# ngrabaskas/Torch-Automatic-Distributed-Neural-Network

Measured on AMD Instinct MI355X. Metric: samples/sec whole-node ResNet-50 DP + GPT-2 PP at 1/2/4/8 MI355X; scaling eff, higher is better.
Workload: dtype bf16

## Files before the change

madnn/models/resnet.py:

```python
from __future__ import annotations

import os
from typing import List, Optional, Type

import torch
from torch import nn

from ..nn.conv import FusedConv2d
from ..nn.norm import FusedBatchNorm2d as BN
from ..nn.norm import FusedGlobalAvgPool2d, FusedMaxPool2d
from ..ops import (batch_norm_add_bn_relu, bn_relu_conv1x1, bn_relu_conv1x1_epi_supported,
                   bn_relu_conv3x3, conv1x1_route,
                   bn_relu_conv3x3_supported, bn_relu_maxpool, bn_relu_maxpool_supported)

_FORK_DS = os.environ.get("MADNN_FORK_DOWNSAMPLE", "1") != "0"
_DUAL_BN = os.environ.get("MADNN_DUAL_BN", "1") != "0"
_DS_SUB = os.environ.get("MADNN_DS_SUB", "1") != "0"


def conv3x3(cin, cout, stride=1, groups=1, dilation=1):
    return FusedConv2d(cin, cout, 3, stride=stride, padding=dilation, groups=groups, bias=False, dilation=dilation)


def conv1x1(cin, cout, stride=1):
    return FusedConv2d(cin, cout, 1, stride=stride, bias=False)


class BasicBlock(nn.Module):
    expansion = 1

    def __init__(self, inplanes, planes, stride=1, downsample=None):
        super().__init__()
        self.conv1 = conv3x3(inplanes, planes, stride)
        self.bn1 = BN(planes)
        self.conv2 = conv3x3(planes, planes)
# ... 22 lines not shown
        self.downsample = downsample

    def forward(self, x):
        if self.downsample is None:
            y, st, idt = self.conv1(x, stats=True, fork=True)
            if isinstance(idt, torch.Tensor) and isinstance(self.bn3, BN) and self.conv1._k9(x) \
                    and conv1x1_route(x.size(1), self.conv1.weight.size(0))[1] == "k9":
                idt._madnn_defer_mask = True
        elif _FORK_DS:
            dual = self._dual_bn()
            sub = dual and _DS_SUB and isinstance(x, torch.Tensor) and self.downsample[0].subsampled_ok()
            y, st, xf = self.conv1(x, stats=True, fork=2 if sub else True)
            if dual:
                yd, std = (self.downsample[0].forward_subsampled(xf, stats=True) if sub
                           else self.downsample[0](xf, stats=True))
                y, st = self._bn1_conv2(y, st)
                y, st = self._bn2_conv3(y, st)
                return batch_norm_add_bn_relu(y, yd, self.bn3, self.downsample[1], st, std)
            idt = self.downsample(xf)
        else:
            idt = self.downsample(x)
            y, st = self.conv1(x, stats=True)
        y, st = self._bn1_conv2(y, st)
        y, st = self._bn2_conv3(y, st)
        return self.bn3(y, residual=idt, relu=True, stats=st)

    def _bn1_conv2(self, y, st):
        if isinstance(y, torch.Tensor) and isinstance(self.bn1, BN) and isinstance(self.conv2, FusedConv2d) \
                and self.conv2._k13(y) \
                and bn_relu_conv3x3_supported(y, self.bn1, self.conv2.weight):
            return bn_relu_conv3x3(y, self.bn1, self.conv2.weight, stats_in=st, stats=True)
        out = self.bn1(y, relu=True, stats=st)
        return self.conv2(out, stats=True)

    def _bn2_conv3(self, y, st):
        if isinstance(y, torch.Tensor) and isinstance(self.bn2, BN) and isinstance(self.conv3, FusedConv2d) \
                and self.conv3._k9(y) and bn_relu_conv1x1_epi_supported(y, self.bn2, self.conv3.weight):
            return bn_relu_conv1x1(y, self.bn2, self.conv3.weight, stats_in=st, stats=True)
        out = self.bn2(y, relu=True, stats=st)
        return self.conv3(out, stats=True)

    def _dual_bn(self) -> bool:
        ds = self.downsample
        return (_DUAL_BN and isinstance(ds, nn.Sequential) and len(ds) == 2
                and isinstance(ds[0], FusedConv2d) and isinstance(ds[1], BN) and isinstance(self.bn3, BN))

# ... 82 lines not shown
```

madnn/ops/__init__.py:

```python
from __future__ import annotations

import os
import threading
from pathlib import Path
from typing import Optional, Sequence

import torch
import torch.nn.functional as F

from . import reference

HERE = Path(__file__).resolve().parent
_KERNELS = HERE / "_madnn_kernels.so"
_lock = threading.Lock()
_loaded = {"kernels": False, "error": None}


def kernels_path() -> Path:
    return _KERNELS


class StaleKernelsError(RuntimeError):
    """The in-tree kernel library was built from different sources than the tree holds."""

# ... 708 lines not shown


def bn_relu_conv1x1(y: torch.Tensor, bn, w: torch.Tensor, *, stats_in: Optional[torch.Tensor] = None,
                    stats: bool = False):
    if bn_relu_conv1x1_epi_supported(y, bn, w):
        _need_native("bn_relu_conv1x1")
        out, part = _BNReluConv1x1EpiFn.apply(y, w, bn.weight, bn.bias, bn, stats_in, stats)
        return (out, part if part.numel() else None) if stats else out
    a = bn(y, relu=True, stats=stats_in) if _is_fused_bn(bn) else torch.relu(bn(y))
    if conv1x1_supported(a, w):
        return conv1x1(a, w, stats=stats)
    out = torch.nn.functional.conv2d(a, w.view(w.size(0), -1, 1, 1)) if a.dim() == 4 else torch.mm(
        a, w.reshape(w.size(0), -1).t())
    return (out, None) if stats else out


def bn_relu_conv1x1_epi_supported(y: torch.Tensor, bn, w: torch.Tensor) -> bool:
    return (_BN_DGRAD_EPI and isinstance(y, torch.Tensor) and bn.training and bn.track_running_stats
            and bn.affine and bn.momentum is not None and bn.weight.dtype == torch.float32
            and conv1x1_supported(y, w) and bn_supported(y, bn.weight)
            and conv1x1_route(y.size(1), w.size(0))[1] == "k9")


class _BNReluMaxPoolFn(torch.autograd.Function):

    @staticmethod
    def forward(ctx, y, bn_w, bn_b, bn, stats_in, p):
        mean, invstd, scale, shift = torch.ops.madnn.bn_coef(y, bn_w, bn_b, bn.running_mean, bn.running_var,
                                                             bn.num_batches_tracked, float(bn.momentum),
                                                             float(bn.eps), stats_in)
        out, arg = torch.ops.madnn.pool_bn_fwd(y, scale, shift, int(p))
        ctx.save_for_backward(y, arg, bn_w, mean, invstd, scale, shift)
        ctx.p = int(p)
        return out

    @staticmethod
    def backward(ctx, dp):
        y, arg, bn_w, mean, invstd, scale, shift = ctx.saved_tensors
        dy, dw, db = torch.ops.madnn.pool_bn_bwd(dp, arg, y, bn_w, mean, invstd, scale, shift, ctx.p)
        return dy, dw, db, None, None, None


def bn_relu_maxpool_supported(y: torch.Tensor, bn, pool) -> bool:
    def pair(v):
        return tuple(v) if isinstance(v, (tuple, list)) else (v, v)
    return (_POOL_BN and isinstance(y, torch.Tensor) and y.device.type == "cuda" and y.dtype == torch.bfloat16 and y.dim() == 4
# ... 211 lines not shown
        if ctx.needs_input_grad[1]:
            dw = torch.ops.madnn.stem_wgrad(dy, x).to(w.dtype)
            if not dw.is_contiguous(memory_format=torch.contiguous_format) or w.stride() != dw.stride():
                dw = torch.empty_like(w).copy_(dw)
        return dx, dw, None


def stem_conv(x: torch.Tensor, w: torch.Tensor, *, stats: bool = False):
    _need_native("stem_conv")
    y, part = _StemFn.apply(x, w, stats)
    return (y, part) if stats else y


def hidden_supported(h: int) -> bool:
    return h % 8 == 0 and h <= 16384


__all__ = [
    "bucket_pack", "bucket_unpack", "flat_scale_cast", "sgd_step", "adam_step", "grad_norm", "layer_norm",
    "rms_norm", "batch_norm_act", "bn_supported", "cross_entropy", "attention", "attention_qkvpacked", "attention_supported",
    "max_pool2d", "max_pool_supported", "conv1x1", "conv1x1_route", "batch_norm_add_bn_relu",
    "batch_norm_dual_supported", "bn_relu_conv1x1", "bn_relu_maxpool",
    "bn_relu_maxpool_supported", "bn_relu_conv3x3", "bn_relu_conv3x3_supported",
    "bn_relu_conv1x1_epi_supported", "conv1x1_supported", "stem_conv", "stem_supported", "native_available", "load_kernels", "kernels_path", "hidden_supported", "reference",
]

if os.environ.get("MADNN_EAGER_LOAD", "0") == "1":
    load_kernels()


FUSED_LINEAR = os.environ.get("MADNN_FUSED_LINEAR", "1") != "0"

def _gelu_tanh_grad(p: torch.Tensor) -> torch.Tensor:
    k0, k1 = 0.7978845608028654, 0.044715
    t = torch.tanh(k0 * (p + k1 * p * p * p))
    return 0.5 * (1 + t) + 0.5 * p * (1 - t * t) * k0 * (1 + 3 * k1 * p * p)


GELU_KIND = {"tanh": 1, "none": 2}


def _gelu_grad_ref(p: torch.Tensor, kind: int) -> torch.Tensor:
    if kind == 1:
        return _gelu_tanh_grad(p)
    cdf = 0.5 * (1.0 + torch.erf(p * 0.7071067811865476))
    return cdf + p * torch.exp(-0.5 * p * p) * 0.3989422804014327

# ... 548 lines not shown
```

madnn/ops/csrc/binding.cpp:

```cpp
#include <torch/library.h>
#include <ATen/ATen.h>
#include <ATen/hip/impl/HIPGuardImplMasqueradingAsCUDA.h>
#include <ATen/hip/impl/HIPStreamMasqueradingAsCUDA.h>
#include <hip/hip_runtime.h>

#include <vector>

#include "attn.h"

extern "C" {
hipError_t madnn_bucket_pack(void* const*, const int64_t*, const int64_t*, int, void*, int, int, float, hipStream_t);
hipError_t madnn_bucket_unpack(void* const*, const int64_t*, const int64_t*, int, void*, int, int, float, hipStream_t);
hipError_t madnn_flat_scale_cast(const void*, void*, int64_t, int, int, float, hipStream_t);
hipError_t madnn_sgd_step(float*, const void*, int, float*, void*, int, int64_t, float, float, float, float, int, int,
                          float, const float*, hipStream_t);
hipError_t madnn_adam_step(float*, const void*, int, float*, float*, void*, int, int64_t, float, float, float, float,
                           float, int, float, float, float, const float*, hipStream_t);
int madnn_sqnorm_grid(int64_t);
hipError_t madnn_sqnorm_partial(const void*, int, int64_t, float, float*, int, hipStream_t);
hipError_t madnn_norm_finalize(const float*, int, float, float*, hipStream_t);
hipError_t madnn_norm_fwd(const void*, const void*, const void*, const void*, void*, void*, float*, float*, int64_t,
                          int, float, int, int, int, hipStream_t);
int64_t madnn_norm_bwd_workspace(int64_t, int);
hipError_t madnn_norm_bwd(const void*, const void*, const void*, const float*, const float*, const void*, void*, void*,
// ... 24 lines not shown
hipError_t madnn_pool_bn_bwd(const void*, const void*, const void*, const float*, const float*, const float*,
                             const float*, const float*, void*, float*, float*, float*, float*, int, int, int, int, int,
                             int, int, hipStream_t);
hipError_t madnn_maxpool_bwd(const void*, const void*, void*, int, int, int, int, int, int, int, int, int, int,
                             hipStream_t);
hipError_t madnn_xent_fwd(const void*, int, const int64_t*, int64_t, int64_t, int64_t, int, int, float*, float*,
                          hipStream_t);
hipError_t madnn_xent_bwd(const void*, int, const int64_t*, const float*, int64_t, int64_t, int64_t, int, int, int64_t,
                          const float*, void*, hipStream_t);
int madnn_xent_fused_chunks(int64_t);
hipError_t madnn_xent_fused(const void*, int, const int64_t*, int64_t, int64_t, int64_t, int, int, int64_t,
                            const float*, float*, void*, hipStream_t);
hipError_t madnn_xent_rescale(void*, int, int64_t, const float*, hipStream_t);
hipError_t madnn_bn_bwd(const void*, const void*, const unsigned char*, int, void*, void*, int64_t, int, int, int,
                        const float*, const float*, const float*, const float*, const float*, float*, float*, float*,
                        float*, hipStream_t);
hipError_t madnn_bn_fwd_dual(const void*, const void*, void*, unsigned char*, int64_t, int, float, float, const float*,
                             const float*, float*, float*, int64_t*, float*, float*, float*, float*, const float*, int,
                             float, float, const float*, const float*, float*, float*, int64_t*, float*, float*,
                             float*, float*, const float*, int, float*, hipStream_t);
hipError_t madnn_bn_bwd_dual(const void*, const void*, const void*, const unsigned char*, void*, void*, int64_t, int,
                             const float*, const float*, const float*, const float*, const float*, const float*,
                             float*, float*, float*, float*, float*, float*, hipStream_t);
int madnn_conv1x1_supported(int64_t, int64_t);
int madnn_conv1x1_stat_rows(int64_t, int64_t, int64_t);
hipError_t madnn_conv1x1_fwd(const void*, const void*, void*, float*, int64_t, int64_t, int64_t, hipStream_t);
hipError_t madnn_conv1x1_dgrad(const void*, const void*, void*, const void*, int64_t, int64_t, int64_t, const void*,
                               const float*, const float*, float*, hipStream_t, const unsigned char* = nullptr);
int madnn_conv1x1_dgrad_rows(int64_t, int64_t, int64_t);
int64_t madnn_conv1x1_wgrad_ws(int64_t, int64_t, int64_t);
hipError_t madnn_conv1x1_wgrad(const void*, const void*, void*, int, float*, int64_t, int64_t, int64_t, hipStream_t);
hipError_t madnn_bn_coef(const void*, int64_t, int, float, float, const float*, const float*, float*, float*, int64_t*,
                         float*, float*, float*, float*, float*, const float*, int, hipStream_t);
int madnn_stem_supported(int, int);
int madnn_stem_stat_rows(int, int, int);
hipError_t madnn_stem_fwd(const void*, const void*, void*, float*, int, int, int, hipStream_t);
int64_t madnn_stem_wgrad_ws(int, int, int);
hipError_t madnn_stem_wgrad(const void*, const void*, float*, float*, int, int, int, hipStream_t);
int madnn_gemm_supported(int64_t, int64_t, int64_t, int64_t, int64_t);
int madnn_conv3x3_supported(int, int, int, int);
int madnn_conv3x3_stat_rows(int64_t);
hipError_t madnn_conv3x3_fwd(const void*, const void*, void*, float*, int, int, int, int, int, hipStream_t);
int madnn_conv3x3_s2_supported(int, int, int, int);
int madnn_conv3x3_s2_stat_rows(int, int, int);
hipError_t madnn_conv3x3_fwd_s2(const void*, const void*, void*, float*, int, int, int, int, int, hipStream_t);
int64_t madnn_conv3x3_wgrad_ws(int, int, int, int, int);
// ... 528 lines not shown
  at::hip::HIPGuardMasqueradingAsCUDA guard(dy.device());
  at::Tensor dx = conv_out_like(dy, cin);
  at::Tensor part = at::empty({madnn_conv1x1_dgrad_rows(M, cin, cout), 2, cin}, dy.options().dtype(at::kFloat));
  check(madnn_conv1x1_dgrad(dy.data_ptr(), w.data_ptr(), dx.data_ptr(), nullptr, M, cin, cout, bny.data_ptr(),
                            scale.data_ptr<float>(), shift.data_ptr<float>(), part.data_ptr<float>(), cur_stream(dy)),
        "conv1x1_dgrad_bnb");
  return {dx, part};
}

at::Tensor conv1x1_wgrad(const at::Tensor& dy, const at::Tensor& x, bool out_bf16) {
  const int64_t cout = dy.size(1), cin = x.size(1);
  const int64_t M = conv_rows(x, cin, "x");
  TORCH_CHECK(conv_rows(dy, cout, "dy") == M && dy.dim() == x.dim(), "conv1x1_wgrad: dy / x pixel mismatch");
  TORCH_CHECK(madnn_conv1x1_supported(cin, cout), "conv1x1: channels must be multiples of 64");
  at::hip::HIPGuardMasqueradingAsCUDA guard(x.device());
  at::Tensor dw = at::empty({cout, cin}, x.options().dtype(out_bf16 ? at::kBFloat16 : at::kFloat));
  at::Tensor ws = at::empty({madnn_conv1x1_wgrad_ws(M, cin, cout)}, x.options().dtype(at::kFloat));
  check(madnn_conv1x1_wgrad(dy.data_ptr(), x.data_ptr(), dw.data_ptr(), out_bf16 ? 1 : 0, ws.data_ptr<float>(), M, cin,
                            cout, cur_stream(x)),
        "conv1x1_wgrad");
  return dw;
}

void gemm_check(const at::Tensor& t, const char* name) {
  check_dev(t, name);
  TORCH_CHECK(t.scalar_type() == at::kBFloat16, "linear: ", name, " must be bf16");
  TORCH_CHECK(t.is_contiguous(), "linear: ", name, " must be contiguous");
  TORCH_CHECK(reinterpret_cast<uintptr_t>(t.data_ptr()) % 16 == 0, "linear: ", name, " must be 16-B aligned");
}

std::tuple<at::Tensor, at::Tensor> linear_fwd(const at::Tensor& x, const at::Tensor& w,
                                              const c10::optional<at::Tensor>& bias,
                                              const c10::optional<at::Tensor>& res, int64_t act, bool save_aux) {
  gemm_check(x, "x");
  gemm_check(w, "w");
  const int64_t K = x.size(-1), N = w.size(0), M = x.numel() / std::max<int64_t>(K, 1);
  TORCH_CHECK(w.dim() == 2 && w.size(1) == K, "linear: weight must be [N, K]");
  TORCH_CHECK(madnn_gemm_supported(N, M, K, K, K), "linear: unsupported shape M=", M, " N=", N, " K=", K);
  at::hip::HIPGuardMasqueradingAsCUDA guard(x.device());
  std::vector<int64_t> shape(x.sizes().begin(), x.sizes().end());
  shape.back() = N;
  at::Tensor y = at::empty(shape, x.options());
  at::Tensor aux = save_aux ? at::empty(shape, x.options()) : at::empty({0}, x.options());
  const bool hb = bias.has_value() && bias->defined();
  if (hb) {
    check_dev(*bias, "bias");
// ... 719 lines not shown
      "bn_bwd(Tensor dy, Tensor x, Tensor? mask, bool has_res, Tensor? w, Tensor save_mean, Tensor save_invstd, "
      "Tensor scale, Tensor shift, bool relu, bool need_wgrad, bool write_dres=True) -> (Tensor, Tensor, Tensor, Tensor)");
  m.def(
      "bn_fwd_dual(Tensor x, Tensor r, Tensor? w, Tensor? b, Tensor(a!)? run_mean, Tensor(b!)? run_var, "
      "Tensor(c!)? nbt, float momentum, float eps, Tensor? partial, Tensor? w_r, Tensor? b_r, "
      "Tensor(d!)? run_mean_r, Tensor(e!)? run_var_r, Tensor(f!)? nbt_r, float momentum_r, float eps_r, "
      "Tensor? partial_r) -> Tensor[]");
  m.def(
      "bn_bwd_dual(Tensor dy, Tensor x, Tensor r, Tensor mask, Tensor? w, Tensor save_mean, Tensor save_invstd, "
      "Tensor? w_r, Tensor save_mean_r, Tensor save_invstd_r) -> Tensor[]");
  m.def("attn_fwd(Tensor q, Tensor k, Tensor v, bool causal, float scale) -> (Tensor, Tensor)");
  m.def(
      "attn_bwd(Tensor dout, Tensor q, Tensor k, Tensor v, Tensor o, Tensor lse, Tensor(a!) dq, Tensor(b!) dk, "
      "Tensor(c!) dv, bool causal, float scale, Tensor(d!)? colsum=None) -> ()");
  m.def("conv1x1_fwd(Tensor x, Tensor w, bool stats) -> (Tensor, Tensor)");
  m.def("conv1x1_dgrad(Tensor dy, Tensor w, Tensor? res=None, Tensor? resmask=None) -> Tensor");
  m.def("conv1x1_dgrad_bnb(Tensor dy, Tensor w, Tensor bny, Tensor scale, Tensor shift) -> (Tensor, Tensor)");
  m.def(
      "conv3x3_fwd_bnb(Tensor x, Tensor w, Tensor bny, Tensor scale, Tensor shift) -> (Tensor, Tensor)");
  m.def(
      "bn_bwd_ext(Tensor dy, Tensor x, Tensor? w, Tensor save_mean, Tensor save_invstd, Tensor scale, Tensor shift, "
      "Tensor partial, bool relu) -> (Tensor, Tensor, Tensor)");
  m.def("conv1x1_wgrad(Tensor dy, Tensor x, bool out_bf16=False) -> Tensor");
  m.def(
      "bn_coef(Tensor x, Tensor? w, Tensor? b, Tensor(a!)? run_mean, Tensor(b!)? run_var, Tensor(c!)? nbt, "
      "float momentum, float eps, Tensor? partial=None) -> Tensor[]");
  m.def("stem_fwd(Tensor x, Tensor wp, bool stats) -> (Tensor, Tensor)");
  m.def("linear_fwd(Tensor x, Tensor w, Tensor? bias, Tensor? res, int act, bool save_aux) -> (Tensor, Tensor)");
  m.def("linear_dgrad(Tensor dy, Tensor w, Tensor? res, bool accumulate) -> Tensor");
  m.def("linear_wgrad(Tensor dy, Tensor x, Tensor? out, bool accumulate, int splits) -> Tensor");
  m.def("linear_wgrad4(Tensor dy, Tensor x, Tensor? out, bool accumulate, int splits) -> Tensor");
  m.def("linear_wgrad4h(Tensor dy, Tensor x, Tensor? out, bool accumulate, int splits) -> Tensor");
  m.def("wgrad_splits(int M, int N, int K) -> int", &wgrad_splits);
  m.def("gemmp_supported(int I, int J, int K, bool has_bias) -> bool", &gemmp_supported);
  m.def("linear_fwd_p(Tensor x, Tensor w, Tensor? bias, int act) -> (Tensor, Tensor)");
  m.def("linear_dgrad_p(Tensor dy, Tensor w, Tensor? pre, ScalarType bias_dtype, int gelu_kind=1) -> (Tensor, Tensor)");
  m.def("conv3x3_fwd(Tensor x, Tensor w, bool stats) -> (Tensor, Tensor)");
  m.def("conv3x3_fwd_s2(Tensor x, Tensor w, bool stats) -> (Tensor, Tensor)");
  m.def("conv3x3_wgrad(Tensor dy, Tensor x, bool out_bf16) -> Tensor");
  m.def("stem_wgrad(Tensor dy, Tensor x) -> Tensor");
  m.def("bias_grad(Tensor dy, Tensor? pre, ScalarType bias_dtype, int gelu_kind=1) -> (Tensor, Tensor)");
  m.def("gelu_fwd(Tensor x, int kind=1) -> Tensor");
  m.def("rope_qkv_(Tensor(a!) qkv, Tensor cos, Tensor sin, int rot_heads, bool inverse) -> Tensor(a!)");
  m.def("rope_qkv(Tensor qkv, Tensor cos, Tensor sin, int rot_heads, bool inverse) -> Tensor");
  m.def("swiglu_fwd(Tensor gu) -> Tensor");
  m.def("swiglu_bwd(Tensor dh, Tensor gu) -> Tensor");
// ... 36 lines not shown
  m.impl("conv3x3_fwd_bnb", conv3x3_fwd_bnb);
  m.impl("conv1x1_dgrad_bnb", conv1x1_dgrad_bnb);
  m.impl("bn_bwd_ext", bn_bwd_ext);
  m.impl("bn_bwd_dual", bn_bwd_dual);
  m.impl("xent_fwd", xent_fwd);
  m.impl("xent_bwd", xent_bwd);
  m.impl("xent_fused", xent_fused);
  m.impl("xent_rescale", xent_rescale);
  m.impl("maxpool_fwd", maxpool_fwd);
  m.impl("pool_bn_fwd", pool_bn_fwd);
  m.impl("pool_bn_bwd", pool_bn_bwd);
  m.impl("bias_grad", bias_grad);
  m.impl("gelu_fwd", gelu_fwd);
  m.impl("rope_qkv_", rope_qkv_);
  m.impl("rope_qkv", rope_qkv);
  m.impl("swiglu_fwd", swiglu_fwd);
  m.impl("swiglu_bwd", swiglu_bwd);
  m.impl("attn_fwd", attn_fwd);
  m.impl("attn_bwd", attn_bwd);
  m.impl("maxpool_bwd", maxpool_bwd);
  m.impl("conv1x1_fwd", conv1x1_fwd);
  m.impl("conv1x1_dgrad", conv1x1_dgrad);
  m.impl("conv1x1_wgrad", conv1x1_wgrad);
  m.impl("stem_fwd", stem_fwd);
  m.impl("stem_wgrad", stem_wgrad);
  m.impl("linear_fwd", linear_fwd);
  m.impl("linear_dgrad", linear_dgrad);
  m.impl("linear_wgrad", linear_wgrad);
  m.impl("linear_wgrad4", linear_wgrad4);
  m.impl("linear_wgrad4h", linear_wgrad4h);
  m.impl("linear_fwd_p", linear_fwd_p);
  m.impl("linear_dgrad_p", linear_dgrad_p);
  m.impl("conv3x3_fwd", conv3x3_fwd);
  m.impl("conv3x3_fwd_s2", conv3x3_fwd_s2);
  m.impl("conv3x3_wgrad", conv3x3_wgrad);
  m.impl("hwq_wait", hwq_wait);
  m.impl("hwq_set", hwq_set);
  m.impl("hwq_batch", hwq_batch);
  m.impl("hwq_spin", hwq_spin);
}
```

madnn/ops/csrc/bn.hip:

```cpp
#include <type_traits>

#include "common.h"

namespace madnn {

constexpr int kBnThreads = 256;
constexpr int kFinSlices = 32;

struct BnGeom {
  int tpr, rpi;
};

struct BnTune {
  int reverse = 1;
  int wg_per_cu = 3;
  int hoist = 1;
  int partials_per_cu = 2;
};
inline BnTune& bn_tune() {
  static BnTune t;
  return t;
}
inline int bn_walk_flags() { return (bn_tune().reverse ? 1 : 0) | (bn_tune().hoist ? 0 : 2); }

// ... 501 lines not shown
      part = prereduce(ext_partial, G, C, ps, qo, workspace, stream);
    } else {
      MADNN_DISPATCH_DT(xdt, XDT, {
        hipLaunchKernelGGL((bn_stats_kernel<XDT>), dim3(G), dim3(kBnThreads), lds, stream, x, M, C, workspace);
      });
      MADNN_HIP_CHECK(hipGetLastError());
    }
    hipLaunchKernelGGL(bn_stats_finalize_kernel, dim3((C + 31) / 32), dim3(32 * kFinSlices), 0, stream, part, G, C, M, eps,
                       momentum, w, b, save_mean, save_invstd, scale, shift, run_mean, run_var, nbt);
  } else {
    hipLaunchKernelGGL(bn_eval_coef_kernel, dim3((C + 255) / 256), dim3(256), 0, stream, C, eps, w, b, run_mean,
                       run_var, scale, shift);
  }
  MADNN_HIP_CHECK(hipGetLastError());
  const int64_t total = M * C;
  const int grid = stream_grid(total, 256 * 8, bn_tune().wg_per_cu * kNumCU);
  MADNN_DISPATCH_DT(xdt, XDT, MADNN_BN_VARIANT(relu, res != nullptr, RELU, RES, {
    hipLaunchKernelGGL((bn_apply_kernel<XDT, RELU, RES>), dim3(grid), dim3(256), 0, stream, x, res, scale, shift, y,
                       mask, total, C, bn_walk_flags());
  }));
  return hipGetLastError();
}

hipError_t madnn_bn_bwd(const void* dy, const void* x, const unsigned char* mask, int has_res, void* dx, void* dres,
                        int64_t M, int C, int xdt, int relu, const float* w, const float* save_mean,
                        const float* save_invstd, const float* scale, const float* shift, float* dw, float* db,
                        float* coef, float* workspace, hipStream_t stream) {
  using namespace madnn;
  if (!madnn_bn_supported(C)) return hipErrorInvalidValue;
  if (M <= 0) return hipSuccess;
  const int G = bn_grid_rows(M, C);
  const BnGeom g = bn_geom(C);
  const size_t lds = g.rpi > 1 ? (size_t)g.rpi * 2 * C * sizeof(float) : 0;
  if (relu && has_res && mask == nullptr) return hipErrorInvalidValue;
  MADNN_DISPATCH_DT(xdt, XDT, MADNN_BN_VARIANT(relu, has_res, RELU, RES, {
    hipLaunchKernelGGL((bn_bwd_reduce_kernel<XDT, RELU, RELU && RES>), dim3(G), dim3(kBnThreads), lds, stream, dy, x,
                       mask, scale, shift, M, C, workspace);
  }));
  MADNN_HIP_CHECK(hipGetLastError());
  float* ca = coef;
  float* cb = coef + C;
  float* cc = coef + 2 * C;
  hipLaunchKernelGGL(bn_bwd_finalize_kernel, dim3((C + 31) / 32), dim3(32 * kFinSlices), 0, stream, workspace, G, C, 2 * C, C, M, w,
                     save_mean, save_invstd, dw, db, ca, cb, cc);
  MADNN_HIP_CHECK(hipGetLastError());
  const int64_t total = M * C;
  const int grid = stream_grid(total, 256 * 8, bn_tune().wg_per_cu * kNumCU);
  MADNN_DISPATCH_DT(xdt, XDT, MADNN_BN_VARIANT(relu, has_res, RELU, RES, {
    hipLaunchKernelGGL((bn_bwd_apply_kernel<XDT, RELU, RES>), dim3(grid), dim3(256), 0, stream, dy, x, mask, scale,
                       shift, ca, cb, cc, dx, dres, total, C, bn_walk_flags());
  }));
  return hipGetLastError();
}


hipError_t madnn_bn_fwd_dual(const void* x, const void* r, void* y, unsigned char* mask, int64_t M, int C,
                             float eps, float momentum, const float* w, const float* b, float* run_mean,
                             float* run_var, int64_t* nbt, float* save_mean, float* save_invstd, float* scale,
                             float* shift, const float* ext_partial, int ext_rows, float eps_r, float momentum_r,
                             const float* w_r, const float* b_r, float* run_mean_r, float* run_var_r,
                             int64_t* nbt_r, float* save_mean_r, float* save_invstd_r, float* scale_r,
                             float* shift_r, const float* ext_partial_r, int ext_rows_r, float* workspace,
                             hipStream_t stream) {
  using namespace madnn;
  if (!madnn_bn_supported(C) || mask == nullptr) return hipErrorInvalidValue;
  if (M <= 0) return hipSuccess;
  const BnGeom g = bn_geom(C);
  const size_t lds = g.rpi > 1 ? (size_t)g.rpi * 2 * C * sizeof(float) : 0;
// ... 124 lines not shown
```

madnn/ops/csrc/conv.hip:

```cpp
#include "mfma.h"

namespace madnn {
namespace conv {

using namespace mf;

constexpr int kThreads = 256;
constexpr int kBK = 64;
constexpr int kTargetWG = 2 * kNumCU;

struct Tune {
  int fwd_wg = kTargetWG;
  int wgrad_wg = 2 * kNumCU;
  int xcd = 1;
};
inline Tune& tune() {
  static Tune t;
  return t;
}

enum Mode : int { kStoreT = 0, kSplit = 1 };

struct GemmArgs {
  const uint16_t* a;
// ... 296 lines not shown
  for (int64_t v = (int64_t)blockIdx.x * 256 + threadIdx.x; v < n4; v += (int64_t)gridDim.x * 256) {
    f32x4 acc = reinterpret_cast<const f32x4*>(slab)[v];
    for (int s = 1; s < splits; ++s) acc += reinterpret_cast<const f32x4*>(slab + (int64_t)s * n)[v];
    if constexpr (BF16) {
      const unsigned lo = (unsigned)f32_to_bf16(acc[0]) | ((unsigned)f32_to_bf16(acc[1]) << 16);
      const unsigned hi = (unsigned)f32_to_bf16(acc[2]) | ((unsigned)f32_to_bf16(acc[3]) << 16);
      reinterpret_cast<u32x2*>(dw)[v] = u32x2{lo, hi};
    } else {
      reinterpret_cast<f32x4*>(dw)[v] = acc;
    }
  }
}

inline void wgrad_split(int64_t M, int64_t cin, int64_t cout, int& bi, int& bj, int64_t& tiles, int& k_chunk,
                        int64_t& splits) {
  bi = cout % 128 == 0 ? 128 : 64;
  bj = cin % 128 == 0 ? 128 : 64;
  tiles = (cout / bi) * (cin / bj);
  const int64_t nk = (M + kBK - 1) / kBK;
  splits = (tune().wgrad_wg + tiles - 1) / tiles;
  splits = splits < 1 ? 1 : (splits > nk ? nk : splits);
  k_chunk = (int)((nk + splits - 1) / splits);
  splits = (nk + k_chunk - 1) / k_chunk;
}

}
}

using namespace madnn::conv;

extern "C" {

int madnn_conv1x1_tune(int key, int value) {
  int* f = key == 0 ? &tune().fwd_wg : key == 1 ? &tune().wgrad_wg : key == 2 ? &tune().xcd : nullptr;
  if (f == nullptr) return -1;
  const int old = *f;
  if (value >= 0) *f = value;
  return old;
}

int madnn_conv1x1_supported(int64_t cin, int64_t cout) {
  return (cin % 64 == 0 && cout % 64 == 0 && cin >= 64 && cout >= 64 && cin <= 16384 && cout <= 16384) ? 1 : 0;
}

int madnn_conv1x1_stat_rows(int64_t M, int64_t cin, int64_t cout) {
  if (!madnn_conv1x1_supported(cin, cout) || M <= 0) return 0;
// ... 97 lines not shown
  if (ws == nullptr) return hipErrorInvalidValue;
  p.out = ws;
  p.i_tiles = (int)(cout / bi);
  p.j_tiles = (int)(cin / bj);
  const int grid = (int)(tiles * splits);
  p.j_groups = 0;
  hipError_t e;
  if (bi == 128 && bj == 128) e = launch<true, true, 128, 128, kSplit, false>(p, grid, s);
  else if (bi == 128) e = launch<true, true, 128, 64, kSplit, false>(p, grid, s);
  else if (bj == 128) e = launch<true, true, 64, 128, kSplit, false>(p, grid, s);
  else e = launch<true, true, 64, 64, kSplit, false>(p, grid, s);
  if (e != hipSuccess) return e;
  const int64_t n = cin * cout;
  const int64_t blocks = (n / 4 + 255) / 256;
  const dim3 grid_r((unsigned)(blocks < 4 * madnn::kNumCU ? blocks : 4 * madnn::kNumCU));
  if (dw_bf16) {
    hipLaunchKernelGGL(split_reduce_kernel<true>, grid_r, dim3(256), 0, s, ws, (int)splits, n, dw);
  } else {
    hipLaunchKernelGGL(split_reduce_kernel<false>, grid_r, dim3(256), 0, s, ws, (int)splits, n, dw);
  }
  return hipGetLastError();
}

}
```

Baseline: 13440.

## Fuse bn3 backward apply, conv3 dgrad/wgrad and bn2 stats into one kernel

Adds an autograd function for non-downsample bottleneck blocks with 64->256 channels that chains bn2, conv3 and bn3+residual+ReLU in the forward pass. In the backward pass, a new HIP kernel applies the bn3 backward coefficients to dout on the fly and computes conv3 dgrad and wgrad together from one pass over the tile. It also accumulates the bn2 backward partial sums in its epilogue, so the bn3 dx tensor is never materialised and the separate dgrad, wgrad and stats passes are removed. The cost is a specialised kernel that only handles C=64 (layer1), a per-workgroup fp32 weight-gradient slab buffer that needs a split-reduce, and more complexity in the backward path.

```diff
diff --git a/madnn/models/resnet.py b/madnn/models/resnet.py
--- a/madnn/models/resnet.py
+++ b/madnn/models/resnet.py
@@ -9,8 +9,8 @@
 from ..nn.conv import FusedConv2d
 from ..nn.norm import FusedBatchNorm2d as BN
 from ..nn.norm import FusedGlobalAvgPool2d, FusedMaxPool2d
-from ..ops import (batch_norm_add_bn_relu, bn_relu_conv1x1, bn_relu_conv1x1_epi_supported,
-                   bn_relu_conv3x3, conv1x1_route,
+from ..ops import (batch_norm_add_bn_relu, bn2_conv3_bn3_add_relu, bn2_conv3_bn3_supported, bn_relu_conv1x1,
+                   bn_relu_conv1x1_epi_supported, bn_relu_conv3x3, conv1x1_route,
                    bn_relu_conv3x3_supported, bn_relu_maxpool, bn_relu_maxpool_supported)
 
 _FORK_DS = os.environ.get("MADNN_FORK_DOWNSAMPLE", "1") != "0"
@@ -79,6 +79,10 @@
             idt = self.downsample(x)
             y, st = self.conv1(x, stats=True)
         y, st = self._bn1_conv2(y, st)
+        if self.downsample is None and isinstance(self.bn2, BN) and isinstance(self.bn3, BN) \
+                and isinstance(self.conv3, FusedConv2d) and isinstance(y, torch.Tensor) and self.conv3._k9(y) \
+                and bn2_conv3_bn3_supported(y, self.bn2, self.conv3.weight, self.bn3, idt):
+            return bn2_conv3_bn3_add_relu(y, self.bn2, self.conv3.weight, self.bn3, idt, stats_in=st)
         y, st = self._bn2_conv3(y, st)
         return self.bn3(y, residual=idt, relu=True, stats=st)
 
diff --git a/madnn/ops/__init__.py b/madnn/ops/__init__.py
--- a/madnn/ops/__init__.py
+++ b/madnn/ops/__init__.py
@@ -754,6 +754,63 @@
             and conv1x1_route(y.size(1), w.size(0))[1] == "k9")
 
 
+class _BN2Conv3BN3Fn(torch.autograd.Function):
+
+    @staticmethod
+    def forward(ctx, y2, w3, bn2_w, bn2_b, bn3_w, bn3_b, idt, bn2, bn3, stats_in):
+        a2, mean2, invstd2, scale2, shift2, _ = torch.ops.madnn.bn_fwd(
+            y2, None, bn2_w, bn2_b, bn2.running_mean, bn2.running_var, bn2.num_batches_tracked, True,
+            float(bn2.momentum), float(bn2.eps), True, stats_in)
+        y3, part = torch.ops.madnn.conv1x1_fwd(a2, w3, True)
+        out, mean3, invstd3, scale3, shift3, mask = torch.ops.madnn.bn_fwd(
+            y3, idt, bn3_w, bn3_b, bn3.running_mean, bn3.running_var, bn3.num_batches_tracked, True,
+            float(bn3.momentum), float(bn3.eps), True, part)
+        ctx.save_for_backward(y2, a2, w3, y3, mask, bn2_w, mean2, invstd2, scale2, shift2, bn3_w, mean3, invstd3,
+                              scale3, shift3)
+        return out
+
+    @staticmethod
+    def backward(ctx, dout):
+        (y2, a2, w3, y3, mask, bn2_w, mean2, invstd2, scale2, shift2, bn3_w, mean3, invstd3, scale3,
+         shift3) = ctx.saved_tensors
+        if dout.dtype != y3.dtype or dout.stride() != y3.stride():
+            dout = torch.empty_like(y3).copy_(dout)
+        coef, dbw3, dbb3 = torch.ops.madnn.bn_bwd_coef(dout, y3, mask, bn3_w, mean3, invstd3, scale3, shift3)
+        da2, part, dw3 = torch.ops.madnn.bn3_conv3_bwd(dout, y3, mask, coef, w3, a2, y2, scale2, shift2,
+                                                       w3.dtype == torch.bfloat16)
+        dy2, dbw2, dbb2 = torch.ops.madnn.bn_bwd_ext(da2, y2, bn2_w, mean2, invstd2, scale2, shift2, part, True)
+        dres = dout.view_as(dout)
+        _attach(dres, "_madnn_resmask", mask)
+        need2 = ctx.needs_input_grad[2] or ctx.needs_input_grad[3]
+        need3 = ctx.needs_input_grad[4] or ctx.needs_input_grad[5]
+        return (dy2, dw3.to(w3.dtype).view(w3.shape), dbw2 if need2 else None, dbb2 if need2 else None,
+                dbw3 if need3 else None, dbb3 if need3 else None, dres, None, None, None)
+
+
+_BN3_CONV3_FUSED = os.environ.get("MADNN_BN3_CONV3_FUSED", "1") != "0"
+
+
+def bn2_conv3_bn3_supported(y2: torch.Tensor, bn2, w3: torch.Tensor, bn3, idt: torch.Tensor) -> bool:
+    def ok(m):
+        return (m.training and m.track_running_stats and m.affine and m.momentum is not None
+                and m.weight.dtype == torch.float32)
+    if not (_BN3_CONV3_FUSED and DEFER_RES_MASK and isinstance(y2, torch.Tensor) and isinstance(idt, torch.Tensor)):
+        return False
+    c, c4 = y2.size(1), w3.size(0)
+    return (bn_relu_conv1x1_epi_supported(y2, bn2, w3) and native_available()
+            and bool(torch.ops.madnn.bn3_conv3_bwd_supported(c, c4)) and conv1x1_route(c, c4)[0] == "k9" and ok(bn2) and ok(bn3)
+            and bn3.weight.numel() == c4 and y2.requires_grad and torch.is_grad_enabled()
+            and getattr(idt, "_madnn_defer_mask", False) and idt.dtype == y2.dtype and idt.dim() == y2.dim()
+            and idt.size(1) == c4 and idt.shape[2:] == y2.shape[2:] and idt.size(0) == y2.size(0)
+            and bn_supported(idt, bn3.weight))
+
+
+def bn2_conv3_bn3_add_relu(y2: torch.Tensor, bn2, w3: torch.Tensor, bn3, idt: torch.Tensor,
+                           stats_in: Optional[torch.Tensor] = None) -> torch.Tensor:
+    _need_native("bn2_conv3_bn3_add_relu")
+    return _BN2Conv3BN3Fn.apply(y2, w3, bn2.weight, bn2.bias, bn3.weight, bn3.bias, idt, bn2, bn3, stats_in)
+
+
 class _BNReluMaxPoolFn(torch.autograd.Function):
 
     @staticmethod
@@ -1011,7 +1068,7 @@
     "max_pool2d", "max_pool_supported", "conv1x1", "conv1x1_route", "batch_norm_add_bn_relu",
     "batch_norm_dual_supported", "bn_relu_conv1x1", "bn_relu_maxpool",
     "bn_relu_maxpool_supported", "bn_relu_conv3x3", "bn_relu_conv3x3_supported",
-    "bn_relu_conv1x1_epi_supported", "conv1x1_supported", "stem_conv", "stem_supported", "native_available", "load_kernels", "kernels_path", "hidden_supported", "reference",
+    "bn_relu_conv1x1_epi_supported", "bn2_conv3_bn3_add_relu", "bn2_conv3_bn3_supported", "conv1x1_supported", "stem_conv", "stem_supported", "native_available", "load_kernels", "kernels_path", "hidden_supported", "reference",
 ]
 
 if os.environ.get("MADNN_EAGER_LOAD", "0") == "1":
diff --git a/madnn/ops/csrc/binding.cpp b/madnn/ops/csrc/binding.cpp
--- a/madnn/ops/csrc/binding.cpp
+++ b/madnn/ops/csrc/binding.cpp
@@ -70,6 +70,14 @@
 hipError_t madnn_bn_bwd_dual(const void*, const void*, const void*, const unsigned char*, void*, void*, int64_t, int,
                              const float*, const float*, const float*, const float*, const float*, const float*,
                              float*, float*, float*, float*, float*, float*, hipStream_t);
+hipError_t madnn_bn_bwd_coef(const void*, const void*, const unsigned char*, int, int64_t, int, int, int, const float*,
+                             const float*, const float*, const float*, const float*, float*, float*, float*, float*,
+                             hipStream_t);
+int madnn_bn3_conv3_bwd_supported(int64_t, int64_t);
+int madnn_bn3_conv3_bwd_groups(int64_t);
+hipError_t madnn_bn3_conv3_bwd(const void*, const void*, const unsigned char*, const float*, const void*, const void*,
+                               const void*, const float*, const float*, void*, float*, float*, void*, int, int64_t,
+                               int64_t, int64_t, hipStream_t);
 int madnn_conv1x1_supported(int64_t, int64_t);
 int madnn_conv1x1_stat_rows(int64_t, int64_t, int64_t);
 hipError_t madnn_conv1x1_fwd(const void*, const void*, void*, float*, int64_t, int64_t, int64_t, hipStream_t);
@@ -644,6 +652,65 @@
   return dw;
 }
 
+std::tuple<at::Tensor, at::Tensor, at::Tensor> bn_bwd_coef(const at::Tensor& dy, const at::Tensor& x,
+                                                           const at::Tensor& mask, const c10::optional<at::Tensor>& w,
+                                                           const at::Tensor& save_mean, const at::Tensor& save_invstd,
+                                                           const at::Tensor& scale, const at::Tensor& shift) {
+  check_dev(x, "x");
+  const int64_t C = x.size(1);
+  const int64_t M = bn_rows(x, C);
+  TORCH_CHECK(dy.strides() == x.strides() && dy.scalar_type() == x.scalar_type(), "bn_bwd_coef: dy / x of one layout");
+  TORCH_CHECK(mask.scalar_type() == at::kByte && mask.is_contiguous() && mask.numel() == x.numel() / 8,
+              "bn_bwd_coef: ReLU bit mask required");
+  at::hip::HIPGuardMasqueradingAsCUDA guard(x.device());
+  auto fo = x.options().dtype(at::kFloat);
+  at::Tensor dw = at::empty({C}, fo), db = at::empty({C}, fo), coef = at::empty({3, C}, fo);
+  at::Tensor ws = at::empty({(int64_t)madnn_bn_partial_rows(M, (int)C) * 2 * C}, fo);
+  check(madnn_bn_bwd_coef(dy.data_ptr(), x.data_ptr(), mask.data_ptr<uint8_t>(), 1, M, (int)C, dt_code(x), 1, optf(w),
+                          save_mean.data_ptr<float>(), save_invstd.data_ptr<float>(), scale.data_ptr<float>(),
+                          shift.data_ptr<float>(), dw.data_ptr<float>(), db.data_ptr<float>(), coef.data_ptr<float>(),
+                          ws.data_ptr<float>(), cur_stream(x)),
+        "bn_bwd_coef");
+  return {coef, dw, db};
+}
+
+bool bn3_conv3_bwd_supported(int64_t c, int64_t c4) { return madnn_bn3_conv3_bwd_supported(c, c4) != 0; }
+
+std::tuple<at::Tensor, at::Tensor, at::Tensor> bn3_conv3_bwd(const at::Tensor& dout, const at::Tensor& y3,
+                                                             const at::Tensor& mask, const at::Tensor& coef,
+                                                             const at::Tensor& w3, const at::Tensor& a2,
+                                                             const at::Tensor& y2, const at::Tensor& scale2,
+                                                             const at::Tensor& shift2, bool dw_bf16) {
+  const int64_t c4 = y3.size(1), c = a2.size(1);
+  const int64_t M = conv_rows(y3, c4, "y3");
+  TORCH_CHECK(madnn_bn3_conv3_bwd_supported(c, c4), "bn3_conv3_bwd: unsupported channels ", c, " -> ", c4);
+  TORCH_CHECK(M > 0, "bn3_conv3_bwd: empty input");
+  TORCH_CHECK(conv_rows(dout, c4, "dout") == M && dout.dim() == y3.dim(), "bn3_conv3_bwd: dout layout");
+  TORCH_CHECK(conv_rows(a2, c, "a2") == M && a2.dim() == y3.dim(), "bn3_conv3_bwd: a2 layout");
+  TORCH_CHECK(conv_rows(y2, c, "y2") == M && y2.dim() == y3.dim(), "bn3_conv3_bwd: y2 layout");
+  conv_check_w(w3, c4, c);
+  TORCH_CHECK(mask.scalar_type() == at::kByte && mask.is_contiguous() && mask.numel() == M * c4 / 8,
+              "bn3_conv3_bwd: ReLU bit mask over y3 required");
+  TORCH_CHECK(coef.scalar_type() == at::kFloat && coef.is_contiguous() && coef.numel() == 3 * c4,
+              "bn3_conv3_bwd: fp32 [3, 4C] coefficients");
+  TORCH_CHECK(scale2.numel() == c && shift2.numel() == c && scale2.scalar_type() == at::kFloat &&
+                  shift2.scalar_type() == at::kFloat && scale2.is_contiguous() && shift2.is_contiguous(),
+              "bn3_conv3_bwd: fp32 [C] scale / shift");
+  at::hip::HIPGuardMasqueradingAsCUDA guard(y3.device());
+  auto fo = y3.options().dtype(at::kFloat);
+  const int64_t groups = madnn_bn3_conv3_bwd_groups(M);
+  at::Tensor da2 = conv_out_like(y3, c);
+  at::Tensor part = at::empty({groups, 2, c}, fo);
+  at::Tensor slabs = at::empty({groups, c4, c}, fo);
+  at::Tensor dw = at::empty({c4, c}, y3.options().dtype(dw_bf16 ? at::kBFloat16 : at::kFloat));
+  check(madnn_bn3_conv3_bwd(dout.data_ptr(), y3.data_ptr(), mask.data_ptr<uint8_t>(), coef.data_ptr<float>(),
+                            w3.data_ptr(), a2.data_ptr(), y2.data_ptr(), scale2.data_ptr<float>(),
+                            shift2.data_ptr<float>(), da2.data_ptr(), part.data_ptr<float>(), slabs.data_ptr<float>(),
+                            dw.data_ptr(), dw_bf16 ? 1 : 0, M, c, c4, cur_stream(y3)),
+        "bn3_conv3_bwd");
+  return {da2, part, dw};
+}
+
 void gemm_check(const at::Tensor& t, const char* name) {
   check_dev(t, name);
   TORCH_CHECK(t.scalar_type() == at::kBFloat16, "linear: ", name, " must be bf16");
@@ -1409,6 +1476,13 @@
       "bn_bwd_ext(Tensor dy, Tensor x, Tensor? w, Tensor save_mean, Tensor save_invstd, Tensor scale, Tensor shift, "
       "Tensor partial, bool relu) -> (Tensor, Tensor, Tensor)");
   m.def("conv1x1_wgrad(Tensor dy, Tensor x, bool out_bf16=False) -> Tensor");
+  m.def(
+      "bn_bwd_coef(Tensor dy, Tensor x, Tensor mask, Tensor? w, Tensor save_mean, Tensor save_invstd, Tensor scale, "
+      "Tensor shift) -> (Tensor, Tensor, Tensor)");
+  m.def("bn3_conv3_bwd_supported(int c, int c4) -> bool", &bn3_conv3_bwd_supported);
+  m.def(
+      "bn3_conv3_bwd(Tensor dout, Tensor y3, Tensor mask, Tensor coef, Tensor w3, Tensor a2, Tensor y2, Tensor scale2, "
+      "Tensor shift2, bool dw_bf16) -> (Tensor, Tensor, Tensor)");
   m.def(
       "bn_coef(Tensor x, Tensor? w, Tensor? b, Tensor(a!)? run_mean, Tensor(b!)? run_var, Tensor(c!)? nbt, "
       "float momentum, float eps, Tensor? partial=None) -> Tensor[]");
@@ -1491,6 +1565,8 @@
   m.impl("conv1x1_fwd", conv1x1_fwd);
   m.impl("conv1x1_dgrad", conv1x1_dgrad);
   m.impl("conv1x1_wgrad", conv1x1_wgrad);
+  m.impl("bn_bwd_coef", bn_bwd_coef);
+  m.impl("bn3_conv3_bwd", bn3_conv3_bwd);
   m.impl("stem_fwd", stem_fwd);
   m.impl("stem_wgrad", stem_wgrad);
   m.impl("linear_fwd", linear_fwd);
diff --git a/madnn/ops/csrc/bn.hip b/madnn/ops/csrc/bn.hip
--- a/madnn/ops/csrc/bn.hip
+++ b/madnn/ops/csrc/bn.hip
@@ -547,10 +547,10 @@
   return hipGetLastError();
 }
 
-hipError_t madnn_bn_bwd(const void* dy, const void* x, const unsigned char* mask, int has_res, void* dx, void* dres,
-                        int64_t M, int C, int xdt, int relu, const float* w, const float* save_mean,
-                        const float* save_invstd, const float* scale, const float* shift, float* dw, float* db,
-                        float* coef, float* workspace, hipStream_t stream) {
+hipError_t madnn_bn_bwd_coef(const void* dy, const void* x, const unsigned char* mask, int has_res, int64_t M, int C,
+                             int xdt, int relu, const float* w, const float* save_mean, const float* save_invstd,
+                             const float* scale, const float* shift, float* dw, float* db, float* coef,
+                             float* workspace, hipStream_t stream) {
   using namespace madnn;
   if (!madnn_bn_supported(C)) return hipErrorInvalidValue;
   if (M <= 0) return hipSuccess;
@@ -563,12 +563,23 @@
                        mask, scale, shift, M, C, workspace);
   }));
   MADNN_HIP_CHECK(hipGetLastError());
-  float* ca = coef;
-  float* cb = coef + C;
-  float* cc = coef + 2 * C;
   hipLaunchKernelGGL(bn_bwd_finalize_kernel, dim3((C + 31) / 32), dim3(32 * kFinSlices), 0, stream, workspace, G, C, 2 * C, C, M, w,
-                     save_mean, save_invstd, dw, db, ca, cb, cc);
-  MADNN_HIP_CHECK(hipGetLastError());
+                     save_mean, save_invstd, dw, db, coef, coef + C, coef + 2 * C);
+  return hipGetLastError();
+}
+
+hipError_t madnn_bn_bwd(const void* dy, const void* x, const unsigned char* mask, int has_res, void* dx, void* dres,
+                        int64_t M, int C, int xdt, int relu, const float* w, const float* save_mean,
+                        const float* save_invstd, const float* scale, const float* shift, float* dw, float* db,
+                        float* coef, float* workspace, hipStream_t stream) {
+  using namespace madnn;
+  if (!madnn_bn_supported(C)) return hipErrorInvalidValue;
+  if (M <= 0) return hipSuccess;
+  MADNN_HIP_CHECK(madnn_bn_bwd_coef(dy, x, mask, has_res, M, C, xdt, relu, w, save_mean, save_invstd, scale, shift, dw,
+                                    db, coef, workspace, stream));
+  const float* ca = coef;
+  const float* cb = coef + C;
+  const float* cc = coef + 2 * C;
   const int64_t total = M * C;
   const int grid = stream_grid(total, 256 * 8, bn_tune().wg_per_cu * kNumCU);
   MADNN_DISPATCH_DT(xdt, XDT, MADNN_BN_VARIANT(relu, has_res, RELU, RES, {
diff --git a/madnn/ops/csrc/conv.hip b/madnn/ops/csrc/conv.hip
--- a/madnn/ops/csrc/conv.hip
+++ b/madnn/ops/csrc/conv.hip
@@ -342,6 +342,247 @@
   splits = splits < 1 ? 1 : (splits > nk ? nk : splits);
   k_chunk = (int)((nk + splits - 1) / splits);
   splits = (nk + k_chunk - 1) / k_chunk;
+}
+
+constexpr int kFC = 64, kFC4 = 256, kFBM = 128;
+constexpr int kFW = kFC4 * kFC, kFT = kFBM * 64;
+
+struct FusedArgs {
+  const uint16_t* dout;
+  const uint16_t* y3;
+  const unsigned char* mask;
+  const float* coef;
+  const uint16_t* w3;
+  const uint16_t* a2;
+  const uint16_t* y2;
+  const float* sc2;
+  const float* sh2;
+  uint16_t* da2;
+  float* partial;
+  float* slabs;
+  int64_t M;
+  int m_tiles;
+};
+
+__global__ __launch_bounds__(kThreads, 2) void bn3_conv3_bwd_kernel(const FusedArgs p) {
+  __shared__ __attribute__((aligned(16))) uint16_t smem[kFW + 3 * kFT];
+  uint16_t* const wt = smem;
+  uint16_t* const dyt = smem + kFW;
+  uint16_t* const at = dyt + 2 * kFT;
+  const int tid = threadIdx.x, wave = tid >> 6, lane = tid & 63, l32 = lane & 31, hh = lane >> 5;
+  const int G = gridDim.x;
+  const int c8 = tid & 7, r8 = tid >> 3;
+
+  {
+    Stage<false, kFBM> sw;
+#pragma unroll
+    for (int h = 0; h < kFC4 / kFBM; ++h) {
+      sw.load(p.w3, kFC, h * kFBM, kFC4, 0, kFC, tid);
+      sw.store(wt + h * kFT, tid);
+    }
+  }
+  float ssum[8], ssq[8];
+#pragma unroll
+  for (int e = 0; e < 8; ++e) ssum[e] = ssq[e] = 0.f;
+  f32x16 accw[kFC4 / 64], accd[2];
+#pragma unroll
+  for (int q = 0; q < kFC4 / 64; ++q) accw[q] = zero16();
+  accd[0] = accd[1] = zero16();
+
+  u32x4 sd[4], sy[4], sa[4];
+  unsigned mk[4];
+  auto opaque = [](unsigned v) {
+    asm volatile("" : "+v"(v));
+    return v;
+  };
+  auto row_of = [&](int tile, int i) {
+    const int valid = (int)min((int64_t)kFBM, p.M - (int64_t)tile * kFBM);
+    return min(r8 + 32 * i, valid - 1);
+  };
+  auto load_step = [&](int tile, int q) {
+    const int64_t m0 = (int64_t)tile * kFBM;
+    const char* bd = reinterpret_cast<const char*>(p.dout + m0 * kFC4 + q * 64);
+    const char* by = reinterpret_cast<const char*>(p.y3 + m0 * kFC4 + q * 64);
+    const unsigned char* bm = p.mask + m0 * (kFC4 / 8) + q * 8;
+#pragma unroll
+    for (int i = 0; i < 4; ++i) {
+      const unsigned r = (unsigned)row_of(tile, i);
+      const unsigned vo = opaque((r * kFC4 + 8 * c8) * 2u), vm = opaque(r * (kFC4 / 8) + c8);
+      sd[i] = *reinterpret_cast<const u32x4*>(bd + vo);
+      sy[i] = *reinterpret_cast<const u32x4*>(by + vo);
+      mk[i] = (unsigned)(int)reinterpret_cast<const signed char*>(bm)[vm];
+    }
+  };
+  auto load_a2 = [&](int tile) {
+    const char* ba = reinterpret_cast<const char*>(p.a2 + (int64_t)tile * kFBM * kFC);
+#pragma unroll
+    for (int i = 0; i < 4; ++i)
+      sa[i] = *reinterpret_cast<const u32x4*>(ba + opaque(((unsigned)row_of(tile, i) * kFC + 8 * c8) * 2u));
+  };
+  auto store_a2 = [&]() {
+    char* a0 = reinterpret_cast<char*>(at) + opaque((unsigned)swz<64>(r8, c8));
+#pragma unroll
+    for (int i = 0; i < 4; ++i) *reinterpret_cast<u32x4*>(a0 + 4096 * i) = sa[i];
+  };
+  auto convert_store = [&](uint16_t* tile_lds, int tile, int q) {
+    const float* cf = p.coef + q * 64 + 8 * c8;
+    f32x4 ca[2], cb[2], cc[2];
+#pragma unroll
+    for (int h = 0; h < 2; ++h) {
+      ca[h] = *reinterpret_cast<const f32x4*>(cf + 4 * h);
+      cb[h] = *reinterpret_cast<const f32x4*>(cf + kFC4 + 4 * h);
+      cc[h] = *reinterpret_cast<const f32x4*>(cf + 2 * kFC4 + 4 * h);
+    }
+    __builtin_amdgcn_sched_barrier(0);
+    const int valid = (int)min((int64_t)kFBM, p.M - (int64_t)tile * kFBM);
+    unsigned mb[4];
+#pragma unroll
+    for (int i = 0; i < 4; ++i) mb[i] = opaque(mk[i]);
+    u32x4 o[4];
+#pragma unroll
+    for (int i = 0; i < 4; ++i) {
+      const unsigned keep = r8 + 32 * i < valid ? 0xffffffffu : 0u;
+#pragma unroll
+      for (int e = 0; e < 4; ++e) {
+        float v[2];
+#pragma unroll
+        for (int hf = 0; hf < 2; ++hf) {
+          const int k = 2 * e + hf;
+          const float d = bf16_to_f32((unsigned short)(hf ? sd[i][e] >> 16 : sd[i][e] & 0xffffu));
+          const float y = bf16_to_f32((unsigned short)(hf ? sy[i][e] >> 16 : sy[i][e] & 0xffffu));
+          const float g = ((mb[i] >> k) & 1u) ? d : 0.f;
+          v[hf] = ca[k >> 2][k & 3] * g + cb[k >> 2][k & 3] * y + cc[k >> 2][k & 3];
+        }
+        o[i][e] = ((unsigned)f32_to_bf16(v[0]) | ((unsigned)f32_to_bf16(v[1]) << 16)) & keep;
+      }
+    }
+    char* t0 = reinterpret_cast<char*>(tile_lds) + opaque((unsigned)swz<64>(r8, c8));
+#pragma unroll
+    for (int i = 0; i < 4; ++i) *reinterpret_cast<u32x4*>(t0 + 4096 * i) = o[i];
+  };
+  auto out_off = [](int r, int c) { return r * 128 + 16 * (c ^ ((r >> 1) & 7)); };
+
+  int tile = blockIdx.x;
+  load_step(tile, 0);
+  load_a2(tile);
+  convert_store(dyt, tile, 0);
+  store_a2();
+  __syncthreads();
+  int cur = 0;
+  for (;;) {
+    const int ntile = tile + G;
+    const bool more = ntile < p.m_tiles;
+#pragma unroll
+    for (int q = 0; q < kFC4 / 64; ++q) {
+      const bool last = q == kFC4 / 64 - 1;
+      const int nq = last ? 0 : q + 1;
+      const int nt = last ? ntile : tile;
+      const bool go = !last || more;
+      if (go) {
+        load_step(nt, nq);
+        if (last) load_a2(nt);
+      }
+      uint16_t* buf = dyt + cur * kFT;
+#pragma unroll
+      for (int s = 0; s < 4; ++s) {
+        const bf16x8 bv = lds_row(buf, wave * 32 + l32, 2 * s + hh);
+#pragma unroll
+        for (int a = 0; a < 2; ++a) accd[a] = mfma(lds_col<64>(wt, q * 64 + 16 * s, a * 32, lane), bv, accd[a]);
+        if (s & 1) __builtin_amdgcn_sched_barrier(0);
+      }
+#pragma unroll
+      for (int s = 0; s < kFBM / 16; ++s) {
+        accw[q] = mfma(lds_col<64>(buf, 16 * s, (wave >> 1) * 32, lane), lds_col<64>(at, 16 * s, (wave & 1) * 32, lane),
+                       accw[q]);
+        if (s & 1) __builtin_amdgcn_sched_barrier(0);
+      }
+      if (go) convert_store(dyt + (cur ^ 1) * kFT, nt, nq);
+      if (last) {
+        __syncthreads();
+        if (more) store_a2();
+        char* ot = reinterpret_cast<char*>(buf);
+        const int jr = (int)opaque((unsigned)(wave * 32 + l32));
+#pragma unroll
+        for (int a = 0; a < 2; ++a)
+#pragma unroll
+          for (int g = 0; g < 4; ++g) {
+            const int ic = a * 32 + 8 * g + 4 * hh;
+            const unsigned lo = (unsigned)f32_to_bf16(accd[a][4 * g]) | ((unsigned)f32_to_bf16(accd[a][4 * g + 1]) << 16);
+            const unsigned hi =
+                (unsigned)f32_to_bf16(accd[a][4 * g + 2]) | ((unsigned)f32_to_bf16(accd[a][4 * g + 3]) << 16);
+            *reinterpret_cast<u32x2*>(ot + out_off(jr, ic >> 3) + 8 * ((ic >> 2) & 1)) = u32x2{lo, hi};
+          }
+        accd[0] = accd[1] = zero16();
+        __syncthreads();
+        float bs[8], bh[8];
+#pragma unroll
+        for (int e = 0; e < 8; ++e) {
+          bs[e] = p.sc2[8 * c8 + e];
+          bh[e] = p.sh2[8 * c8 + e];
+        }
+        const int64_t m0 = (int64_t)tile * kFBM;
+        const int valid = (int)min((int64_t)kFBM, p.M - m0);
+        char* bo = reinterpret_cast<char*>(p.da2 + m0 * kFC);
+        const char* by2 = reinterpret_cast<const char*>(p.y2 + m0 * kFC);
+#pragma unroll
+        for (int u = 0; u < 4; ++u) {
+          const int r = r8 + 32 * u;
+          if (r < valid) {
+            const unsigned off = opaque(((unsigned)r * kFC + 8 * c8) * 2u);
+            const u32x4 v = *reinterpret_cast<const u32x4*>(ot + opaque((unsigned)out_off(r8, c8)) + 4096 * u);
+            *reinterpret_cast<u32x4*>(bo + off) = v;
+            const u32x4 yv = *reinterpret_cast<const u32x4*>(by2 + off);
+#pragma unroll
+            for (int e = 0; e < 4; ++e) {
+#pragma unroll
+              for (int hf = 0; hf < 2; ++hf) {
+                const int k = 2 * e + hf;
+                const float g = bf16_to_f32((unsigned short)(hf ? v[e] >> 16 : v[e] & 0xffffu));
+                const float yy = bf16_to_f32((unsigned short)(hf ? yv[e] >> 16 : yv[e] & 0xffffu));
+                const float gm = yy * bs[k] + bh[k] > 0.f ? g : 0.f;
+                ssum[k] += gm;
+                ssq[k] += gm * yy;
+              }
+            }
+          }
+        }
+      }
+      if (!go) break;
+      __syncthreads();
+      cur ^= 1;
+    }
+    if (!more) break;
+    tile = ntile;
+  }
+
+  const int t2 = (int)opaque(threadIdx.x), w2 = t2 >> 6, col2 = t2 & 31, h2 = (t2 >> 5) & 1;
+  float* slab = p.slabs + (int64_t)blockIdx.x * kFW;
+#pragma unroll
+  for (int q = 0; q < kFC4 / 64; ++q)
+#pragma unroll
+    for (int r = 0; r < 16; ++r)
+      slab[(q * 64 + (w2 >> 1) * 32 + acc_row(r, h2)) * kFC + (w2 & 1) * 32 + col2] = accw[q][r];
+  __syncthreads();
+  float* red = reinterpret_cast<float*>(dyt);
+  const int rg = t2 >> 3, cg = t2 & 7;
+#pragma unroll
+  for (int e = 0; e < 8; ++e) {
+    red[(rg * 2) * kFC + 8 * cg + e] = ssum[e];
+    red[(rg * 2 + 1) * kFC + 8 * cg + e] = ssq[e];
+  }
+  __syncthreads();
+  if (t2 < 2 * kFC) {
+    const int which = t2 / kFC, ii = t2 % kFC;
+    float v = 0.f;
+    for (int g = 0; g < 32; ++g) v += red[(g * 2 + which) * kFC + ii];
+    p.partial[((int64_t)blockIdx.x * 2 + which) * kFC + ii] = v;
+  }
+}
+
+inline int fused_groups(int64_t M) {
+  const int64_t tiles = (M + kFBM - 1) / kFBM;
+  const int64_t want = tune().fwd_wg < 1 ? 1 : tune().fwd_wg;
+  return (int)(tiles < want ? tiles : want);
 }
 
 }
@@ -485,4 +726,42 @@
   return hipGetLastError();
 }
 
-}
+int madnn_bn3_conv3_bwd_supported(int64_t c, int64_t c4) { return (c == kFC && c4 == kFC4) ? 1 : 0; }
+
+int madnn_bn3_conv3_bwd_groups(int64_t M) { return M > 0 ? fused_groups(M) : 0; }
+
+hipError_t madnn_bn3_conv3_bwd(const void* dout, const void* y3, const unsigned char* mask, const float* coef,
+                               const void* w3, const void* a2, const void* y2, const float* sc2, const float* sh2,
+                               void* da2, float* partial, float* slabs, void* dw, int dw_bf16, int64_t M, int64_t c,
+                               int64_t c4, hipStream_t s) {
+  if (!madnn_bn3_conv3_bwd_supported(c, c4) || M <= 0) return hipErrorInvalidValue;
+  FusedArgs p{};
+  p.dout = static_cast<const uint16_t*>(dout);
+  p.y3 = static_cast<const uint16_t*>(y3);
+  p.mask = mask;
+  p.coef = coef;
+  p.w3 = static_cast<const uint16_t*>(w3);
+  p.a2 = static_cast<const uint16_t*>(a2);
+  p.y2 = static_cast<const uint16_t*>(y2);
+  p.sc2 = sc2;
+  p.sh2 = sh2;
+  p.da2 = static_cast<uint16_t*>(da2);
+  p.partial = partial;
+  p.slabs = slabs;
+  p.M = M;
+  p.m_tiles = (int)((M + kFBM - 1) / kFBM);
+  const int grid = fused_groups(M);
+  hipLaunchKernelGGL(bn3_conv3_bwd_kernel, dim3(grid), dim3(kThreads), 0, s, p);
+  hipError_t e = hipGetLastError();
+  if (e != hipSuccess) return e;
+  const int64_t n = kFW;
+  const dim3 grid_r((unsigned)((n / 4 + 255) / 256));
+  if (dw_bf16) {
+    hipLaunchKernelGGL(split_reduce_kernel<true>, grid_r, dim3(256), 0, s, slabs, grid, n, dw);
+  } else {
+    hipLaunchKernelGGL(split_reduce_kernel<false>, grid_r, dim3(256), 0, s, slabs, grid, n, dw);
+  }
+  return hipGetLastError();
+}
+
+}
```

Result: faster. 13910 (median of 6 runs) (+3.5%).
